# ShingoNishimoto/gnss_sim_receiver

Measured on AMD Instinct MI355X. Metric: IF Msamples/sec processed & tracked-channels sustained @1/2/4/8 GPU, higher is better.
Workload: dtype f32

## Files before the change

gnss_sim_receiver_amd/csrc/trk_fast.hip:

```cpp
#include <algorithm>
#include <cstdlib>
#include <type_traits>

#include "code_bits.h"
#include "corr_device.h"
#include "trk_engine.h"

#ifdef GNSSHIP_CORR_PROFILE
namespace gnsship {
namespace {
constexpr int kFProfEpochs = 16;
constexpr int kFProfFirst = 8;
constexpr int kFProfSlots = 88;
__device__ unsigned long long* g_trkf_prof = nullptr;
__shared__ int g_fprof_epoch;
__shared__ unsigned long long g_fprof_lds[kFProfEpochs * kFProfSlots];
#ifndef GNSSHIP_PROF_MASK
#define GNSSHIP_PROF_MASK 0xffffffffffffffffull
#endif
__device__ __forceinline__ constexpr bool prof_on(int k) { return ((GNSSHIP_PROF_MASK) >> (k < 63 ? k : 63)) & 1ull; }
__device__ __forceinline__ void trkf_prof_stamp(int e, int k)
{
    if (!prof_on(k)) return;
    const int r = e - kFProfFirst;
// ... 48 lines not shown
#pragma clang fp contract(off)

namespace gnsship {
namespace {

#ifndef GNSSHIP_FAST_WAVES
#define GNSSHIP_FAST_WAVES 8
#endif
#ifndef GNSSHIP_THRU_WAVES
#define GNSSHIP_THRU_WAVES 6
#endif
#ifndef GNSSHIP_FAST_WAVES_LONG
#define GNSSHIP_FAST_WAVES_LONG 8
#endif
constexpr int kFWaves = GNSSHIP_FAST_WAVES;
constexpr int kFWavesLong = GNSSHIP_FAST_WAVES_LONG;
constexpr int kLongEpoch = 10000;
#ifndef GNSSHIP_PRE_DISC
#define GNSSHIP_PRE_DISC 1
#endif
#ifndef GNSSHIP_ROLE_PLAN_LONG
#define GNSSHIP_ROLE_PLAN_LONG 3
#endif
#ifndef GNSSHIP_ROLE_PLAN
#define GNSSHIP_ROLE_PLAN 0
#endif
template <int NTT>
constexpr int acc_waves() { return (2 * NTT + 3) / 4; }
template <int NTT, int W>
constexpr int n_producers() { return W - 2 - acc_waves<NTT>(); }
constexpr int kMaxAccWaves = 4;
static_assert(kFWaves - 4 >= 1 && GNSSHIP_THRU_WAVES - 4 >= 1, "trk_fast needs at least one producer wave");
constexpr int kRoleControl = 0, kRoleReplay = 1, kRoleProducer = 2, kRoleAccum = 3;
#define GNSSHIP_PROBE(NAME)                                                  \
    do {                                                                     \
        _Pragma("unroll") for (int pr_ = 0; pr_ < (NAME); pr_++) __builtin_amdgcn_s_sleep(4); \
    } while (0)
#ifndef GNSSHIP_DELAY_ACC
#define GNSSHIP_DELAY_ACC 0
#endif
#ifndef GNSSHIP_DELAY_PROD
#define GNSSHIP_DELAY_PROD 0
#endif
#ifndef GNSSHIP_DELAY_REPLAY
#define GNSSHIP_DELAY_REPLAY 0
#endif
#ifndef GNSSHIP_DELAY_LOOP
#define GNSSHIP_DELAY_LOOP 0
#endif
#ifndef GNSSHIP_POLL_SLEEP
#define GNSSHIP_POLL_SLEEP 0
#endif
constexpr uint64_t kSlotEmpty = ~0ull;

struct FJob {
    int64_t off;
    float rem_code, code_step;
    float shifts[5];
    float dz_re, dz_im;
    float rem_carr, step;
    int32_t runnable, in_margin, M, S, tail, steady;
    int32_t narrow;
};

typedef uint32_t u4v __attribute__((ext_vector_type(4)));
constexpr uint32_t kJobRunnable = 1u, kJobInMargin = 2u, kJobSteady = 4u, kJobNarrow = 8u;
struct alignas(16) FJobLds {
    uint32_t w[8];
};
__device__ __forceinline__ void job_store_a(FJobLds& s, int64_t off, uint32_t flags, float rem_code, float code_step)
{
    const uint64_t o = static_cast<uint64_t>(off);
    *reinterpret_cast<u4v*>(&s.w[0]) = u4v{static_cast<uint32_t>(o), (static_cast<uint32_t>(o >> 32) & 0x00ffffffu) | (flags << 24),
        __builtin_bit_cast(uint32_t, rem_code), __builtin_bit_cast(uint32_t, code_step)};
}
__device__ __forceinline__ void job_store_b(FJobLds& s, float rem_carr, float step, float dz_re, float dz_im)
{
    *reinterpret_cast<u4v*>(&s.w[4]) = u4v{__builtin_bit_cast(uint32_t, rem_carr), __builtin_bit_cast(uint32_t, step),
        __builtin_bit_cast(uint32_t, dz_re), __builtin_bit_cast(uint32_t, dz_im)};
}
__device__ __forceinline__ void job_store_carr(FJobLds& s, float rem_carr, float step) { *reinterpret_cast<f2*>(&s.w[4]) = f2{rem_carr, step}; }
__device__ __forceinline__ void job_store_dz(FJobLds& s, f2 dz) { *reinterpret_cast<f2*>(&s.w[6]) = dz; }

struct SpecArgs {
    double step_d, rate;
    int64_t if_num;
    float rem_prev;
    int32_t n_pred;
};

struct alignas(16) SpecPred {
    float rem, step, dz_re, dz_im;
};

struct FShared {
    FJobLds job;
    float taps[2][2 * kMaxTaps + 2];
    int32_t taps_seq[kMaxAccWaves];
    gnsship_trk_dump_record drec;
    double coh;
    int32_t seed_seq;
    int32_t job_seq;
    int32_t pre_seq;
    int32_t lock_seq;
    int32_t locked;
    int32_t tail_seq;
// ... 98 lines not shown
            GNSSHIP_PSTEP_ASM(GNSSHIP_PSTEP("%[x]", "%[w]") GNSSHIP_PSTEP("%[w]", "%[x]"));
    } else if constexpr (N == 3) {
        if constexpr (STORE)
            GNSSHIP_PSTEP_ASM(GNSSHIP_PSTEP("%[x]", "%[w]") GNSSHIP_ST GNSSHIP_PSTEP("%[w]", "%[v]") GNSSHIP_PSTEP("%[v]", "%[x]"));
        else
            GNSSHIP_PSTEP_ASM(GNSSHIP_PSTEP("%[x]", "%[w]") GNSSHIP_PSTEP("%[w]", "%[v]") GNSSHIP_PSTEP("%[v]", "%[x]"));
    } else {
        if constexpr (STORE)
            GNSSHIP_PSTEP_ASM(GNSSHIP_PSTEP("%[x]", "%[w]") GNSSHIP_ST GNSSHIP_PSTEP("%[w]", "%[v]") GNSSHIP_PSTEP("%[v]", "%[w]")
                    GNSSHIP_PSTEP("%[w]", "%[x]"));
        else
            GNSSHIP_PSTEP_ASM(GNSSHIP_PSTEP("%[x]", "%[w]") GNSSHIP_PSTEP("%[w]", "%[v]") GNSSHIP_PSTEP("%[v]", "%[w]") GNSSHIP_PSTEP("%[w]", "%[x]"));
    }
    return x;
}
#undef GNSSHIP_ST
#undef GNSSHIP_PSTEP_ASM

#define GNSSHIP_PS(A, B) GNSSHIP_PSTEP("%[" #A "]", "%[" #B "]")
#define GNSSHIP_TST(A, OFF) "ds_write_b32 %[p], %[" #A "] offset:" #OFF "\n\t"
#define GNSSHIP_TASK8(A, B, OFF)                                                                                            \
    GNSSHIP_PS(A, B) GNSSHIP_TST(A, OFF) GNSSHIP_PS(B, A) GNSSHIP_PS(A, B) GNSSHIP_PS(B, A) GNSSHIP_PS(A, B) GNSSHIP_PS(B, A) \
        GNSSHIP_PS(A, B) GNSSHIP_PS(B, A)
__device__ __forceinline__ float pblock64_g8(float x, float c, float k2, uint32_t lds_off)
{
    float t, u, w;
    asm volatile(GNSSHIP_PS(x, w) GNSSHIP_PS(w, x) GNSSHIP_PS(x, w) GNSSHIP_PS(w, x) GNSSHIP_PS(x, w) GNSSHIP_PS(w, x)
                     GNSSHIP_PS(x, w) GNSSHIP_TASK8(w, x, 128) GNSSHIP_TASK8(w, x, 256) GNSSHIP_TASK8(w, x, 384) GNSSHIP_TASK8(w, x, 512)
                         GNSSHIP_TASK8(w, x, 640) GNSSHIP_TASK8(w, x, 768) GNSSHIP_TASK8(w, x, 896) "v_mov_b32 %[x], %[w]\n\t"
                 : [x] "+v"(x), [t] "=&v"(t), [u] "=&v"(u), [w] "=&v"(w)
                 : [c] "s"(c), [k2] "v"(k2), [p] "v"(lds_off)
                 : "memory");
    return x;
}
#undef GNSSHIP_TST
#undef GNSSHIP_TASK8
#undef GNSSHIP_PS
template <int N>
__device__ __forceinline__ float ppow(float x, float c, float k2)
{
    if constexpr (N >= 4) return ppow<N - 4>(pstep<4, false>(x, c, k2, 0), c, k2);
    else if constexpr (N > 0) return pstep<N, false>(x, c, k2, 0);
    else return x;
}
#undef GNSSHIP_PSTEP

__device__ __forceinline__ float pnormalise(float x)
{
    const float s = __fmul_rn(x, x);
    const float o = __builtin_bit_cast(float, __builtin_amdgcn_mov_dpp(__builtin_bit_cast(int, s), 0xB1, 0xF, 0xF, false));
    return __fdiv_rn(x, sqrt_rn_f32(__fadd_rn(s, o)));
}

template <int G, bool SRING>
__device__ __forceinline__ float fast_replay(float x, float c, float k2, int M, int S, int tail, uint64_t* __restrict__ Zs, int rs, int lane)
{
    static_assert(G % 4 == 0 && G >= 4 && G <= 64, "task length");
    constexpr int kTB = 64 / G;
    if (S <= 0) return x;
    c = __builtin_bit_cast(float, __builtin_amdgcn_readfirstlane(__builtin_bit_cast(int, c)));
    const uint32_t base = static_cast<uint32_t>(reinterpret_cast<uintptr_t>(Zs)) + 4u * static_cast<uint32_t>(lane);
    uint32_t off = base;
    constexpr uint32_t kSlotRow = kAvxLanes * sizeof(uint64_t);
    uint32_t* const half0 = reinterpret_cast<uint32_t*>(Zs) + lane;
    int ts = 0;
    if constexpr (!SRING) {
        const int full = (S - 1) / kTB;
#pragma unroll 1
        for (int b = 0; b < full; b++) {
            if constexpr (G == 8 && kSlotRow == 128) {
                x = pblock64_g8(pnormalise(pstep<1, true>(x, c, k2, off)), c, k2, off);
                off += kTB * kSlotRow;
            } else {
#pragma unroll
                for (int q = 0; q < kTB; q++) {
                    if (q == 0)
                        x = ppow<G - 1>(pnormalise(pstep<1, true>(x, c, k2, off)), c, k2);
                    else
                        x = ppow<G - 4>(pstep<4, true>(x, c, k2, off), c, k2);
                    off += kSlotRow;
                }
            }
        }
        if (full * kTB < S - 1) {
            x = ppow<G - 1>(pnormalise(pstep<1, true>(x, c, k2, off)), c, k2);
            off += kSlotRow;
#pragma unroll 1
            for (int t = full * kTB + 1; t < S - 1; t++) {
                x = ppow<G - 4>(pstep<4, true>(x, c, k2, off), c, k2);
                off += kSlotRow;
            }
        }
        ts = S - 1;
    } else {
        int t = 0;
        if constexpr (G == 8 && kSlotRow == 128) {
            if (rs % kTB == 0) {
                const int full = (S - 1) / kTB;
#pragma unroll 1
                for (int b = 0; b < full; b++, t += kTB) {
                    const int ts0 = t % rs;
                    if (t >= rs) {
                        bool busy = true;
                        while (busy) {
                            uint32_t v[kTB];
#pragma unroll
                            for (int q = 0; q < kTB; q++) v[q] = __hip_atomic_load(half0 + 2 * kAvxLanes * (ts0 + q), __ATOMIC_RELAXED, __HIP_MEMORY_SCOPE_WORKGROUP);
                            busy = false;
#pragma unroll
                            for (int q = 0; q < kTB; q++) busy = busy || v[q] != ~0u;
                            if (busy) __builtin_amdgcn_s_sleep(GNSSHIP_POLL_SLEEP);
                        }
                    }
                    off = base + static_cast<uint32_t>(ts0) * kSlotRow;
                    x = pblock64_g8(pnormalise(pstep<1, true>(x, c, k2, off)), c, k2, off);
                }
            }
        }
        ts = t % rs;
        off = base + static_cast<uint32_t>(ts) * kSlotRow;
#pragma unroll 1
        for (; t < S - 1; t++) {
            if (t >= rs)
                while (__hip_atomic_load(half0 + 2 * kAvxLanes * ts, __ATOMIC_RELAXED, __HIP_MEMORY_SCOPE_WORKGROUP) != ~0u) __builtin_amdgcn_s_sleep(GNSSHIP_POLL_SLEEP);
            if (t % kTB == 0)
                x = ppow<G - 1>(pnormalise(pstep<1, true>(x, c, k2, off)), c, k2);
            else
                x = ppow<G - 4>(pstep<4, true>(x, c, k2, off), c, k2);
            ts = ts + 1 == rs ? 0 : ts + 1;
            off = base + static_cast<uint32_t>(ts) * kSlotRow;
        }
        if (S - 1 >= rs)
            while (__hip_atomic_load(half0 + 2 * kAvxLanes * ts, __ATOMIC_RELAXED, __HIP_MEMORY_SCOPE_WORKGROUP) != ~0u) __builtin_amdgcn_s_sleep(GNSSHIP_POLL_SLEEP);
    }
    __hip_atomic_store(half0 + 2 * kAvxLanes * ts, __builtin_bit_cast(uint32_t, x), __ATOMIC_RELAXED, __HIP_MEMORY_SCOPE_WORKGROUP);
    if (tail > 0) {
        for (int m = G * (S - 1); m < M; m++) {
            x = pstep<1, false>(x, c, k2, 0);
// ... 10 lines not shown
{
    if constexpr (PACKED) return code_chip<IN_MARGIN>(code, L, sn, sh, rem);
    else return code_at<IN_MARGIN>(code, L, sn, sh, rem);
}
__host__ __device__ constexpr int fast_code_stride(bool packed, int code_cap_floats)
{
    return packed ? (lane_code_words(code_cap_floats) + 3) / 4 * 4 : code_cap_floats;
}

template <int NT, bool DATA, bool IN_MARGIN, int G, bool FULL, bool PACKED>
__device__ __forceinline__ void group_codes(CodePtr<PACKED> __restrict__ code0, CodePtr<PACKED> __restrict__ code1, int L, int n0, int cnt, float step,
    float rem, const float (&shifts)[NT], float (&cv)[G][NT + (DATA ? 1 : 0)])
{
    float fn = static_cast<float>(n0);
    const float fn0 = fn;
#pragma unroll
    for (int i = 0; i < G; i++) {
        const bool on = FULL || i < cnt;
        const float sn = __fmul_rn(step, on ? fn : fn0);
#pragma unroll
        for (int q = 0; q < NT; q++) cv[i][q] = chip_at<PACKED, IN_MARGIN>(code0, L, sn, shifts[q], rem);
        if constexpr (DATA) cv[i][NT] = chip_at<PACKED, IN_MARGIN>(code1, L, sn, 0.0f, rem);
        fn += static_cast<float>(kAvxLanes);
    }
}

typedef float f4 __attribute__((ext_vector_type(4)));

template <int NTT, int G>
struct ProdLayout {
    static constexpr int kJ = 4 * G;
    static constexpr int kRow = kJ + 4;
    static constexpr int kSlot = kAvxLanes * kRow;
    static constexpr int kGroup = 2 * NTT * kSlot;
};

template <int NTT, int G, bool FULL, class PL>
__device__ __forceinline__ void store_products4(float* __restrict__ pdst, int i0, int cnt, const f2 (&a)[4], const float (&cv)[G][NTT])
{
    f4 q[2 * NTT];
#pragma unroll
    for (int u = 0; u < 4; u++) {
        const bool on = FULL || i0 + u < cnt;
#pragma unroll
        for (int t = 0; t < NTT; t++) {
            q[2 * t][u] = on ? __fmul_rn(a[u].x, cv[i0 + u][t]) : -0.0f;
            q[2 * t + 1][u] = on ? __fmul_rn(a[u].y, cv[i0 + u][t]) : -0.0f;
        }
    }
#pragma unroll
    for (int sl = 0; sl < 2 * NTT; sl++) *reinterpret_cast<f4*>(pdst + sl * PL::kSlot + i0) = q[sl];
}

template <int FMT, int NTT, int G, bool FULL, class PL>
__device__ __forceinline__ void group_phasors(i4v span, f2 z, f2 dz, bool renorm, int n0, int cnt, float* __restrict__ pdst, const float (&cv)[G][NTT],
    f2 (&xa)[G < 8 ? G : 8], f2 (&xb)[G < 8 ? G : 8])
{
    constexpr int SB = sample_bytes<FMT>();
    constexpr int kB = G < 8 ? G : 8;
    static_assert(kB % 4 == 0, "16-byte product stores");
#pragma unroll 1
    for (int i0 = 0; i0 < G; i0 += kB) {
        if (i0 + kB < G) {
#pragma unroll
            for (int u = 0; u < kB; u++) xb[u] = load_sample<FMT>(span, (n0 + kAvxLanes * (i0 + kB + u)) * SB, 0);
        }
#pragma unroll
        for (int h = 0; h < kB; h += 4) {
            f2 a[4];
#pragma unroll
            for (int u = 0; u < 4; u++) {
                const int i = i0 + h + u;
                a[u] = cmul_exact_pk(xa[h + u], z);
                f2 zn = cmul_exact_s(z, dz);
                if (i == 0 && renorm) zn = normalise_avx(zn);
                z = zn;
            }
            store_products4<NTT, G, FULL, PL>(pdst, i0 + h, cnt, a, cv);
        }
        if (i0 + kB < G) {
#pragma unroll
            for (int u = 0; u < kB; u++) xa[u] = xb[u];
        }
    }
}

template <int FMT, int NT, bool DATA, bool IN_MARGIN, int G, int W, bool PACKED>
__device__ __forceinline__ void fast_produce(const FJob& job, i4v span, CodePtr<PACKED> __restrict__ code0, CodePtr<PACKED> __restrict__ code1, int L,
    uint64_t* __restrict__ Zs, int rs, float* __restrict__ Pp, int rg, int32_t* ready, const int32_t* acc_groups, int gbase, int lane, int pw, int pe,
    f2 (&xa)[G < 8 ? G : 8], float (&cv)[G][NT + (DATA ? 1 : 0)])
{
    constexpr int SB = sample_bytes<FMT>();
    constexpr int NTT = NT + (DATA ? 1 : 0);
    constexpr int NP = n_producers<NTT, W>();
    constexpr int NA = acc_waves<NTT>();
    using PL = ProdLayout<NTT, G>;
    constexpr int kB = G < 8 ? G : 8;
    const int M = job.M, S = job.S;
    const int n_groups = (S + 3) / 4;
    const f2 dz = f2{job.dz_re, job.dz_im};
    const float step = job.code_step, rem = job.rem_code;
    float shifts[NT];
#pragma unroll
    for (int q = 0; q < NT; q++) shifts[q] = job.shifts[q];
    const int tl = lane >> 4, l = lane & (kAvxLanes - 1);
    f2 xb[kB];
    int rslot = pw % rg;
    const int rstep = NP % rg;
    unsigned long long w_ring = 0, w_slot = 0, w_codes = 0, w_prod = 0;
    [[maybe_unused]] const unsigned long long t_run = GNSSHIP_FCLOCK();
    for (int g = pw; g < n_groups; g += NP) {
        const int t = 4 * g + tl;
        const bool active = t < S;
        const int m_lo = G * (active ? t : 0);
        const int cnt = active ? min(G, M - m_lo) : 0;
        const int n0 = kAvxLanes * m_lo + l;
        const bool full = 4 * g + 4 <= S && G * (4 * g + 4) <= M;
        const unsigned long long tA = GNSSHIP_FCLOCK();
#pragma unroll
        for (int u = 0; u < kB; u++) xa[u] = load_sample<FMT>(span, (n0 + kAvxLanes * u) * SB, 0);
        if (full)
            group_codes<NT, DATA, IN_MARGIN, G, true, PACKED>(code0, code1, L, n0, G, step, rem, shifts, cv);
        else
            group_codes<NT, DATA, IN_MARGIN, G, false, PACKED>(code0, code1, L, n0, cnt, step, rem, shifts, cv);
#ifdef GNSSHIP_CORR_PROFILE
        for (int i = 0; i < G; i++)
            for (int q = 0; q < NTT; q++) asm volatile("" ::"v"(cv[i][q]));
#endif
        w_codes += GNSSHIP_FCLOCK() - tA;
        const unsigned long long t0 = GNSSHIP_FCLOCK();
        if (g >= rg) {
#pragma unroll
            for (int a = 0; a < NA; a++) lds_wait_ge(acc_groups + a, gbase + g - rg + 1);
        }
        const unsigned long long t1 = GNSSHIP_FCLOCK();
        w_ring += t1 - t0;
        uint64_t* slot = Zs + (active ? t % rs : 0) * kAvxLanes + l;
        uint64_t v = kSlotEmpty;
        if (active) {
            while (static_cast<uint32_t>(v = load_slot(slot)) == ~0u || static_cast<uint32_t>(v >> 32) == ~0u) __builtin_amdgcn_s_sleep(GNSSHIP_POLL_SLEEP);
            store_slot(slot, __builtin_bit_cast(f2, kSlotEmpty));
        }
        w_slot += GNSSHIP_FCLOCK() - t1;
        if (g == pw && pw == 0) GNSSHIP_FSTAMP(pe, 30);
        if (g + NP >= n_groups && pw == 1) GNSSHIP_FSTAMP(pe, 31);
        const f2 z = active ? __builtin_bit_cast(f2, v) : f2{0.0f, 0.0f};
        const bool renorm = ((G * t) & 63) == 0;
        float* pdst = Pp + static_cast<size_t>(rslot) * PL::kGroup + l * PL::kRow + G * tl;
        const unsigned long long tB = GNSSHIP_FCLOCK();
        if (full)
            group_phasors<FMT, NTT, G, true, PL>(span, z, dz, renorm, n0, G, pdst, cv, xa, xb);
        else
            group_phasors<FMT, NTT, G, false, PL>(span, z, dz, renorm, n0, cnt, pdst, cv, xa, xb);
        GNSSHIP_PROBE(GNSSHIP_DELAY_PROD);
        if (lane == 0) lds_release_store(ready + 2 * rslot, gbase + g + 1);
        w_prod += GNSSHIP_FCLOCK() - tB;
        if (g < 8) GNSSHIP_FSTAMP(pe, 48 + g);
        rslot += rstep;
        if (rslot >= rg) rslot -= rg;
    }
    if (pw == 0) {
        GNSSHIP_FVAL(pe, 41, w_ring);
        GNSSHIP_FVAL(pe, 42, w_slot);
        GNSSHIP_FVAL(pe, 43, GNSSHIP_FCLOCK() - t_run);
        GNSSHIP_FVAL(pe, 79, w_codes);
        GNSSHIP_FVAL(pe, 80, w_prod);
    }
}

template <int NTT>
constexpr int acc_slots() { return (2 * NTT + 4 * acc_waves<NTT>() - 1) / (4 * acc_waves<NTT>()); }
template <int NTT>
__device__ __forceinline__ int acc_slot(int a, int r, int k) { return 4 * (a + acc_waves<NTT>() * k) + r; }

template <int NTT, int G>
__device__ __forceinline__ void fast_accumulate(const float* __restrict__ Pp, int rg, const int32_t* ready, int32_t* acc_done, int gbase, int S,
    int lane, int a, float (&acc)[acc_slots<NTT>()], int pe)
{
    using PL = ProdLayout<NTT, G>;
    constexpr int NS = acc_slots<NTT>();
    constexpr int kQ = PL::kJ / 4;
    const int l = lane & (kAvxLanes - 1), r = lane >> 4;
    const int n_groups = (S + 3) / 4;
    int off[NS];
#pragma unroll
    for (int k = 0; k < NS; k++) {
        acc[k] = 0.0f;
        off[k] = min(acc_slot<NTT>(a, r, k), 2 * NTT - 1) * PL::kSlot + l * PL::kRow;
    }
    unsigned long long w_flag = 0;
    [[maybe_unused]] const unsigned long long t_run = GNSSHIP_FCLOCK();
    int rslot = 0;
    for (int g = 0; g < n_groups; g++) {
        const unsigned long long t0 = GNSSHIP_FCLOCK();
        lds_wait_eq(ready + 2 * rslot, gbase + g + 1);
        const float* src = Pp + static_cast<size_t>(rslot) * PL::kGroup;
        f4 v[kQ][NS];
#pragma unroll
        for (int q = 0; q < kQ; q++)
#pragma unroll
            for (int k = 0; k < NS; k++) v[q][k] = *reinterpret_cast<const f4*>(src + off[k] + 4 * q);
        w_flag += GNSSHIP_FCLOCK() - t0;
#pragma unroll
        for (int q = 0; q < kQ; q++)
#pragma unroll
            for (int k = 0; k < NS; k++)
#pragma unroll
                for (int u = 0; u < 4; u++) acc[k] = __fadd_rn(acc[k], v[q][k][u]);
        if (g == 0) GNSSHIP_FSTAMP(pe, 28);
        if (g == n_groups - 1) GNSSHIP_FSTAMP(pe, 29);
#pragma unroll
        for (int k = 0; k < NS; k++) asm volatile("" ::"v"(acc[k]) : "memory");
        GNSSHIP_PROBE(GNSSHIP_DELAY_ACC);
        if (lane == 0) __hip_atomic_store(acc_done, gbase + g + 1, __ATOMIC_RELAXED, __HIP_MEMORY_SCOPE_WORKGROUP);
        rslot = rslot + 1 == rg ? 0 : rslot + 1;
    }
    if (a < 2) {
        GNSSHIP_FVAL(pe, 44 + 2 * a, w_flag);
        GNSSHIP_FVAL(pe, 45 + 2 * a, GNSSHIP_FCLOCK() - t_run);
    }
}

__device__ __forceinline__ float avx_chain_sum(float d)
{
    float s = d + dpp_mov<0x12C>(d);
    s = s + dpp_mov<0x128>(d);
    s = s + dpp_mov<0x124>(d);
    float r = 0.0f + s;
    r = r + dpp_mov<0x101>(s);
    r = r + dpp_mov<0x102>(s);
    r = r + dpp_mov<0x103>(s);
    return r;
}

template <int FMT, int NT, bool DATA, bool IN_MARGIN, bool PACKED>
__device__ __forceinline__ void fast_tail_products(const FJob& job, i4v span, CodePtr<PACKED> __restrict__ code0, CodePtr<PACKED> __restrict__ code1, int L,
    const f2* T, int lane, f2 (*tp)[kMaxTaps + 1])
{
    constexpr int SB = sample_bytes<FMT>();
    if (lane >= job.tail) return;
    const int n = kAvxLanes * job.M + lane;
    const f2 x = load_sample<FMT>(span, n * SB, 0);
    const f2 wo = cmul_exact(x, T[lane]);
    const float sn = __fmul_rn(job.code_step, static_cast<float>(n));
#pragma unroll
    for (int q = 0; q < NT; q++) {
        const float c = chip_at<PACKED, IN_MARGIN>(code0, L, sn, job.shifts[q], job.rem_code);
        tp[lane][q] = wo * f2{c, c};
    }
    if constexpr (DATA) {
        const float c = chip_at<PACKED, IN_MARGIN>(code1, L, sn, 0.0f, job.rem_code);
        tp[lane][NT] = wo * f2{c, c};
    }
}

__device__ __forceinline__ void stage_code_f(float* dst, const CodeDesc& cd, int nthreads)
{
    const int nq = padded_code_quads(cd.len);
    const float4* src = reinterpret_cast<const float4*>(cd.ptr - kCodeMargin);
    float4* d4 = reinterpret_cast<float4*>(dst);
    for (int q = threadIdx.x; q < nq; q += nthreads) d4[q] = src[q];
}

// ... 23 lines not shown
__device__ __forceinline__ void derive_all(float step, float rem, int lane, f2& inc, f2& dz, f2& zinit)
{
    float ss, cs, sr, cr;
    glibc_sincosf(-step, &ss, &cs);
    glibc_sincosf(rem, &sr, &cr);
    inc = f2{cs, ss};
    const f2 p0 = f2{cr, -sr};
    f2 w = p0, z = p0, d = inc;
#pragma unroll
    for (int i = 0; i < kAvxLanes - 1; i++) {
        w = cmul_exact_sc(w, inc);
        if (i < 4) d = cmul_exact_sc(d, d);
        z = i + 1 == (lane >> 1) ? w : z;
    }
    dz = normalise_avx(d);
    zinit = z;
}

__device__ __forceinline__ uint64_t uni64(uint64_t v)
{
    const uint32_t lo = __builtin_amdgcn_readfirstlane(static_cast<uint32_t>(v)), hi = __builtin_amdgcn_readfirstlane(static_cast<uint32_t>(v >> 32));
    return (static_cast<uint64_t>(hi) << 32) | lo;
}

__device__ __forceinline__ f2 derive_chains(float rem, f2 inc, int lane)
{
    float sfn, cfn;
    glibc_sincosf(rem, &sfn, &cfn);
    const f2 p0 = f2{cfn, -sfn};
    f2 w = p0, z = p0;
#pragma unroll
    for (int i = 0; i < kAvxLanes - 1; i++) {
        w = cmul_exact_sc(w, inc);
        z = i + 1 == (lane >> 1) ? w : z;
    }
    return z;
}

template <int FMT, int NT, bool DATA, int G, bool THRU, bool SRING, int W, bool PACKED>
__global__ __launch_bounds__(W * kWave, (fast_waves_per_simd<THRU, W>())) void trk_fast_kernel(const TrkParams* __restrict__ pk, TrkChannel* __restrict__ chans,
    const CodeDesc* __restrict__ codes, int n_codes, const void* __restrict__ samples, uint64_t buf_first, int64_t buf_len, int max_rounds,
    int n_chans, int code_cap_floats, int rs, int rg, gnsship_trk_epoch* __restrict__ rec, gnsship_trk_dump_record* __restrict__ dump,
    gnsship_trk_corr_trace* __restrict__ trace, int* __restrict__ ran_count)
{
    constexpr int NTT = NT + (DATA ? 1 : 0);
    constexpr int kFWaves = W;
    constexpr int kFThreads = kFWaves * kWave;
    static_assert(acc_waves<NTT>() <= kMaxAccWaves && n_producers<NTT, kFWaves>() >= 1, "trk_fast wave roles");
    extern __shared__ __attribute__((aligned(16))) float lds[];
    __shared__ TrkChannel sc;
    __shared__ FShared sh;
    __shared__ int32_t skip;
    __shared__ f2 tailz[kAvxLanes];
    const int ch = blockIdx.x;
    const int tid = threadIdx.x, lane = tid & (kWave - 1), wave = __builtin_amdgcn_readfirstlane(tid >> 6);
    const TrkParams& k = *pk;
    {
        const int* src = reinterpret_cast<const int*>(chans + ch);
        int* dst = reinterpret_cast<int*>(&sc);
        for (int i = tid; i < static_cast<int>(sizeof(TrkChannel) / 4); i += kFThreads) dst[i] = src[i];
    }
    uint64_t* Zs = reinterpret_cast<uint64_t*>(lds);
    float* code0 = reinterpret_cast<float*>(Zs + static_cast<size_t>(rs) * kAvxLanes);
    const int code_stride = fast_code_stride(PACKED, code_cap_floats);
    float* code1 = code0 + code_stride;
    float* Pp = code0 + (DATA ? 2 : 1) * code_stride;
    int32_t* ready = reinterpret_cast<int32_t*>(Pp + static_cast<size_t>(rg) * ProdLayout<NTT, G>::kGroup);
    for (int i = tid; i < rs * kAvxLanes; i += kFThreads) Zs[i] = kSlotEmpty;
    for (int i = tid; i < 2 * rg; i += kFThreads) ready[i] = 0;
    __shared__ int32_t simd_of[kFWaves];
    if (lane == 0) simd_of[wave] = static_cast<int32_t>((__builtin_amdgcn_s_getreg(4 | (31 << 11)) >> 4) & 3);
#ifdef GNSSHIP_CORR_PROFILE
    for (int i = tid; i < kFProfEpochs * kFProfSlots; i += kFThreads) g_fprof_lds[i] = 0;
#endif
    __syncthreads();
    constexpr int NA = acc_waves<NTT>();
    int role = kRoleProducer, pw = 0;
    {
        auto count = [&](int sd) {
            int c = 0;
            for (int w = 0; w < kFWaves; w++) c += (simd_of[w] & 3) == sd ? 1 : 0;
            return c;
        };
        auto assign = [&](int plan) __attribute__((always_inline)) {
            int nacc = 0, nprod = 0, nsimd = 0;
            bool ctl = false, rep = false;
            for (int cc = 1; cc <= kFWaves; cc++)
                for (int sd = 0; sd < 4; sd++) {
                    if (count(sd) != cc) continue;
                    bool first = true;
                    for (int w = 0; w < kFWaves; w++) {
                        if ((simd_of[w] & 3) != sd) continue;
                        int rl, idx = 0;
                        if (plan == 3) {
                            if (nsimd == 0 && !rep) {
                                rl = kRoleReplay;
                                rep = true;
                            } else if (nsimd == 1 && nacc < NA) {
                                rl = kRoleAccum;
                                idx = nacc++;
                            } else if (nsimd == 2 && !ctl) {
                                rl = kRoleControl;
                                ctl = true;
                            } else if (nsimd >= 2 && nacc < NA) {
                                rl = kRoleAccum;
                                idx = nacc++;
                            } else if (nsimd >= 3 && !ctl) {
                                rl = kRoleControl;
                                ctl = true;
                            } else {
                                rl = kRoleProducer;
                                idx = nprod++;
                            }
                        } else if (plan == 2) {
                            if (nsimd == 0 && !rep) {
                                rl = kRoleReplay;
                                rep = true;
                            } else if (nsimd == 0 && !ctl) {
                                rl = kRoleControl;
                                ctl = true;
                            } else if (nsimd >= 1 && nacc < NA) {
// ... 194 lines not shown
        }
    };
    if (role == kRoleControl) make_seed(0);
    int e_done = 0;
    bool cancel = false;
    if (role == kRoleReplay) {
        float shc[5];
        int sh_nw = -1;
        for (int e = 0;; e++) {
            FJob job;
                bool spec = false;
                SpecArgs sp{};
                while (__hip_atomic_load(&sh.seed_seq, __ATOMIC_RELAXED, __HIP_MEMORY_SCOPE_WORKGROUP) < e + 1) {
                    if (__hip_atomic_load(&sh.step_seq, __ATOMIC_RELAXED, __HIP_MEMORY_SCOPE_WORKGROUP) >= e + 1) {
                        sp.step_d = __builtin_bit_cast(double, uni64(__builtin_bit_cast(uint64_t, sh.spec.step_d)));
                        sp.rate = __builtin_bit_cast(double, uni64(__builtin_bit_cast(uint64_t, sh.spec.rate)));
                        sp.if_num = static_cast<int64_t>(uni64(static_cast<uint64_t>(sh.spec.if_num)));
                        sp.rem_prev = __builtin_bit_cast(float, __builtin_amdgcn_readfirstlane(__builtin_bit_cast(int, sh.spec.rem_prev)));
                        sp.n_pred = __builtin_amdgcn_readfirstlane(sh.spec.n_pred);
                        spec = true;
                        break;
                    }
                    __builtin_amdgcn_s_sleep(GNSSHIP_POLL_SLEEP);
                }
                __builtin_amdgcn_fence(__ATOMIC_ACQUIRE, "workgroup");
                GNSSHIP_FSTAMP(e, 0);
    #ifdef GNSSHIP_CORR_PROFILE
                if (lane == 0) g_fprof_epoch = e;
    #endif
                f2 zinit = f2{0.0f, 0.0f}, inc = f2{1.0f, 0.0f}, dz = f2{1.0f, 0.0f};
                float step_pre = 0.0f;
                bool published = false;
                float xl = 0.0f;
                if (spec) step_pre = static_cast<float>(sp.step_d + if_step);
                if (SRING && spec) derive_step(step_pre, inc, dz);
                if (!SRING && spec) {
                    float rem_pred = carr_rem_next(sp.rem_prev, carr_advance(sp.step_d, sp.rate, static_cast<double>(sp.n_pred)));
                    if (has_if) {
                        const int64_t ifn = (sp.if_num + kp.if_mod * static_cast<int64_t>(sp.n_pred)) % kp.fs_int;
                        const double ifc = static_cast<double>(ifn) / static_cast<double>(kp.fs_int);
                        rem_pred = static_cast<float>(fmod_2pi(static_cast<double>(rem_pred) + kTwoPi * ifc));
                    }
                    derive_all(step_pre, rem_pred, lane, inc, dz, zinit);
                    GNSSHIP_FSTAMP(e, 35);
                    GNSSHIP_PROBE(GNSSHIP_DELAY_REPLAY);
                    if (lane == 0) {
                        sh.pred.rem = rem_pred;
                        sh.pred.step = step_pre;
                        sh.pred.dz_re = dz.x;
                        sh.pred.dz_im = dz.y;
                        publish_seq(&sh.pred_seq, e + 1);
                    }
                    xl = (lane & 1) ? zinit.y : zinit.x;
                    if (lane < 2 * kAvxLanes) xl = fast_replay<G, false>(xl, dz.x, (lane & 1) ? dz.y : -dz.y, M, S, tail, Zs, rs, lane);
                    GNSSHIP_FSTAMP(e, 34);
                    wait_seq(&sh.seed_seq, e + 1);
                    const int v = __builtin_amdgcn_readfirstlane(sh.verdict);
                    int status = (v >> 2) == e + 1 ? (v & 3) : 3;
                    if (status == 3) {
                        const FJob sd = read_job(shc, sh_nw);
                        status = 2;
                        if (sd.runnable && __builtin_bit_cast(uint32_t, sd.step) == __builtin_bit_cast(uint32_t, step_pre) &&
                            __builtin_bit_cast(uint32_t, sd.rem_carr) == __builtin_bit_cast(uint32_t, rem_pred)) {
                            if (lane == 0) {
                                job_store_dz(sh.job, dz);
                                publish_seq(&sh.job_seq, e + 1);
                            }
                            status = 1;
                        }
                    }
                    GNSSHIP_FVAL(e, 78, static_cast<unsigned long long>(status));
                    if (status == 1) {
                        published = true;
                    } else {
                        for (int i = lane; i < S * kAvxLanes; i += kWave) Zs[i] = kSlotEmpty;
                    }
                    GNSSHIP_FSTAMP(e, 36);
                }
                if (!published) {
                    wait_seq(&sh.seed_seq, e + 1);
                    const FJob sd = read_job(shc, sh_nw);
                    if (sd.runnable) {
                        if (!(spec && __builtin_bit_cast(uint32_t, sd.step) == __builtin_bit_cast(uint32_t, step_pre))) derive_step(sd.step, inc, dz);
                        zinit = derive_chains(sd.rem_carr, inc, lane);
                        if (lane == 0) job_store_dz(sh.job, dz);
                    }
                    if (lane == 0) publish_seq(&sh.job_seq, e + 1);
                    if (!sd.runnable) break;
                }
                GNSSHIP_FSTAMP(e, 1);
                GNSSHIP_FCLK(e, 12);
                job = read_job(shc, sh_nw);
                if (!published) {
                    xl = (lane & 1) ? zinit.y : zinit.x;
                    if (lane < 2 * kAvxLanes) xl = fast_replay<G, SRING>(xl, job.dz_re, (lane & 1) ? job.dz_im : -job.dz_im, M, S, tail, Zs, rs, lane);
                }
                if (tail > 0) {
                    const i4v span = sample_span<FMT>(samples, job.off, N);
                    const f2 zl = f2{__builtin_bit_cast(float, __builtin_amdgcn_readlane(__builtin_bit_cast(int, xl), 0)),
                        __builtin_bit_cast(float, __builtin_amdgcn_readlane(__builtin_bit_cast(int, xl), 1))};
                    if (lane == 0) {
                        f2 p = normalise_avx(zl);
                        for (int j = 0; j < tail; j++) {
                            tailz[j] = p;
                            p = cmul_exact(p, inc);
                        }
                    }
                    if (job.in_margin)
                        fast_tail_products<FMT, NT, DATA, true, PACKED>(job, span, c0, c1, L, tailz, lane, sh.tailp);
                    else
                        fast_tail_products<FMT, NT, DATA, false, PACKED>(job, span, c0, c1, L, tailz, lane, sh.tailp);
                    if (lane == 0) publish_seq(&sh.tail_seq, e + 1);
                }
                GNSSHIP_FSTAMP(e, 2);
                GNSSHIP_FCLK(e, 13);
        }
    } else if (role == kRoleProducer) {
        f2 xa[G < 8 ? G : 8];
        float cv[G][NTT];
        bool lost = false;
        float shc[5];
        int sh_nw = -1;
        const double coh_steady = k.code_period * static_cast<double>(k.sync[uni(sc.geo)].extend);
        for (int e = 0;; e++) {
            const int gbase = e * n_groups;
            wait_seq(&sh.job_seq, e + 1);
            const FJob job = read_job(shc, sh_nw);
            if (!job.runnable) break;
            const i4v span = sample_span<FMT>(samples, job.off, N);
            if (job.in_margin)
                fast_produce<FMT, NT, DATA, true, G, kFWaves, PACKED>(job, span, c0, c1, L, Zs, rs, Pp, rg, ready, sh.acc_groups, gbase, lane, pw, e, xa, cv);
            else
                fast_produce<FMT, NT, DATA, false, G, kFWaves, PACKED>(job, span, c0, c1, L, Zs, rs, Pp, rg, ready, sh.acc_groups, gbase, lane, pw, e, xa, cv);
            if (pw < 2) GNSSHIP_FSTAMP(e, 3 + pw);
            if (pw == 0) {
                bool locked = true;
                if (kSteadyForm && job.steady) {
#pragma unroll
                    for (int a = 0; a < NA; a++) wait_seq(&sh.taps_seq[a], e + 1);
                    if (lane == 0) {
                        GNSSHIP_FSTAMP(e, 8);
                        if (!lost) {
                            const float* tp = sh.taps[e & 1] + (k.veml ? 2 : 0);
                            sc.p[0] = __fadd_rn(0.0f, __fmul_rn(1.0f, tp[2]));
                            sc.p[1] = __fadd_rn(0.0f, __fmul_rn(1.0f, tp[3]));
                            locked = lock_status(k, sc, coh_steady);
                        }
                        sh.locked = locked ? 1 : 0;
                        GNSSHIP_FSTAMP(e, 26);
                        publish_seq(&sh.lock_seq, e + 1);
                    }
                } else {
                    wait_seq(&sh.pre_seq, e + 1);
                    const double coh = sh.coh;
                    if (lane == 0) {
                        GNSSHIP_FSTAMP(e, 8);
                        locked = !(coh > 0.0 && !lock_status(k, sc, coh));
                        sh.locked = locked ? 1 : 0;
                        GNSSHIP_FSTAMP(e, 26);
                        publish_seq(&sh.lock_seq, e + 1);
                    }
                }
                lost = __builtin_amdgcn_readfirstlane(locked ? 0 : 1) != 0;
            }
        }
    } else if (role == kRoleAccum) {
        float shc[5];
        int sh_nw = -1;
        for (int e = 0;; e++) {
            const int gbase = e * n_groups;
            wait_seq(&sh.job_seq, e + 1);
            const FJob job = read_job(shc, sh_nw);
            if (!job.runnable) break;
            {
                constexpr int NS = acc_slots<NTT>();
                float acc[NS];
                GNSSHIP_FSTAMP(e, 27);
                fast_accumulate<NTT, G>(Pp, rg, ready, &sh.acc_groups[pw], gbase, S, lane, pw, acc, e);
                GNSSHIP_FSTAMP(e, 5);
                const int r = lane >> 4;
    #pragma unroll
                for (int kk = 0; kk < NS; kk++) acc[kk] = avx_chain_sum(acc[kk]);
                if (job.tail > 0) {
                    wait_seq(&sh.tail_seq, e + 1);
                    for (int j = 0; j < job.tail; j++) {
    #pragma unroll
// ... 283 lines not shown
    }
    __syncthreads();
#ifdef GNSSHIP_CORR_PROFILE
    if (g_trkf_prof)
        for (int i = tid; i < kFProfEpochs * kFProfSlots; i += kFThreads) g_trkf_prof[static_cast<size_t>(blockIdx.x) * kFProfEpochs * kFProfSlots + i] = g_fprof_lds[i];
#endif
    {
        const int* src = reinterpret_cast<const int*>(&sc);
        int* dst = reinterpret_cast<int*>(chans + ch);
        for (int i = tid; i < static_cast<int>(sizeof(TrkChannel) / 4); i += kFThreads) dst[i] = src[i];
    }
}

}

#ifdef GNSSHIP_CORR_PROFILE
}
extern "C" int gnsship_debug_trk_fast_profile(void* dev_buf)
{
    return hipMemcpyToSymbol(HIP_SYMBOL(gnsship::g_trkf_prof), &dev_buf, sizeof(void*)) == hipSuccess ? 0 : -3;
}
namespace gnsship {
#endif

static int device_cus()
{
    static int cache[64] = {0};
    int dev = 0;
    if (hipGetDevice(&dev) != hipSuccess || dev < 0 || dev >= 64) return 256;
    if (cache[dev] == 0) {
        int n = 0;
        cache[dev] = (hipDeviceGetAttribute(&n, hipDeviceAttributeMultiprocessorCount, dev) == hipSuccess && n > 0) ? n : 256;
    }
    return cache[dev];
}

static bool fast_thru(int n_chans)
{
    if (const char* env = std::getenv("GNSSHIP_TRK_THRU")) return env[0] == '1';
    return n_chans > device_cus();
}

struct FastPlan {
    size_t bytes = 0;
    int G = 8, rs = 0, rg = 0;
    bool packed = false;
};
#ifndef GNSSHIP_FAST_G
#define GNSSHIP_FAST_G 8
#endif
constexpr int kFastG = GNSSHIP_FAST_G;
constexpr int kFastSlotRingGroups = 16;
constexpr int kFastMinRingGroups = 4;
constexpr size_t kFastMaxSlotBytes = 48 * 1024;
static bool fast_packed_only_layout(const TrkParams& p) { return p.n_taps == 3 && p.jobs_per_channel > 1; }
static bool fast_packed_layout(const TrkParams& p, bool codes_binary)
{
    if (fast_packed_only_layout(p)) return true;
    if (!p.single_code_bits || !codes_binary || p.n_taps != 3 || p.jobs_per_channel > 1) return false;
    const char* env = std::getenv("GNSSHIP_TRK_FAST_PACKED");
    return !(env && env[0] == '0');
}

static FastPlan fast_plan(const TrkParams& p, int code_cap_floats, int n_chans, bool codes_binary)
{
    FastPlan f;
    f.packed = fast_packed_layout(p, codes_binary);
    if (p.n_taps == 5 && fast_thru(n_chans)) return f;
    const int N = static_cast<int>(p.conf.vector_length);
    const int M = N / kAvxLanes;
    const int G = kFastG;
    const int S = std::max(1, (M + G - 1) / G);
    const int n_groups = (S + 3) / 4;
    const int ntt = p.n_taps + (p.jobs_per_channel > 1 ? 1 : 0);
    const size_t codes = static_cast<size_t>(p.jobs_per_channel > 1 ? 2 : 1) * fast_code_stride(f.packed, code_cap_floats) * sizeof(float);
    const size_t slot_b = kAvxLanes * sizeof(uint64_t);
    const size_t group_b = static_cast<size_t>(2 * ntt) * kAvxLanes * (4 * G + 4) * sizeof(float) + 2 * sizeof(int32_t);
    size_t budget = fast_thru(n_chans) ? 72 * 1024 : kTrkPersistMaxLds;
    if (const char* env = std::getenv("GNSSHIP_TRK_FAST_LDS"))
        budget = std::min(budget, static_cast<size_t>(std::atol(env)) * 1024);
    auto fit = [&](int rs) -> int {
        const size_t used = codes + static_cast<size_t>(rs) * slot_b;
        if (used >= budget) return 0;
        const int rg = static_cast<int>(std::min<size_t>((budget - used) / group_b, static_cast<size_t>(n_groups)));
        return rg >= std::min(2, n_groups) ? rg : 0;
    };
    int rs = S, rg = static_cast<size_t>(S) * slot_b <= kFastMaxSlotBytes ? fit(S) : 0;
    if (rg < std::min(n_groups, kFastMinRingGroups) && S > 4 * kFastSlotRingGroups) {
        const int rg2 = std::min(fit(4 * kFastSlotRingGroups), kFastSlotRingGroups);
        if (rg2 > rg) {
            rs = 4 * kFastSlotRingGroups;
            rg = rg2;
        }
    }
    if (rg == 0) return f;
    f.G = G;
    f.rs = rs;
    f.rg = rg;
    f.bytes = codes + static_cast<size_t>(rs) * slot_b + static_cast<size_t>(rg) * group_b;
    return f;
}

bool trk_fast_thru(int n_chans) { return fast_thru(n_chans); }
int trk_device_cus() { return device_cus(); }

bool trk_fast_supported(const TrkParams& p, int code_cap_floats, int n_chans, bool codes_binary)
{
// ... 82 lines not shown
```

Before: 695.5.

## Publish replay-normalised phasors to LDS so producers skip renormalisation

The replay wave now writes its normalised phasor at each 64-iteration block boundary into a new LDS row array (Zn). Producers poll that row at renorm points and take the exact value instead of calling normalise_avx themselves, which takes a sqrt/divide off the producer critical path. In exchange there is extra LDS space, a spin-wait dependency on the replay wave, and extra slot resets. A profiling stamp for the first accumulator groups is also added.

```diff
diff --git a/gnss_sim_receiver_amd/csrc/trk_fast.hip b/gnss_sim_receiver_amd/csrc/trk_fast.hip
--- a/gnss_sim_receiver_amd/csrc/trk_fast.hip
+++ b/gnss_sim_receiver_amd/csrc/trk_fast.hip
@@ -124,6 +124,8 @@
 #define GNSSHIP_POLL_SLEEP 0
 #endif
 constexpr uint64_t kSlotEmpty = ~0ull;
+constexpr size_t kFastMaxSlotBytes = 48 * 1024;
+constexpr int kZnRows = static_cast<int>(kFastMaxSlotBytes / (kAvxLanes * sizeof(uint64_t)) / 8);
 
 struct FJob {
     int64_t off;
@@ -328,9 +330,12 @@
     return __fdiv_rn(x, sqrt_rn_f32(__fadd_rn(s, o)));
 }
 
-template <int G, bool SRING>
-__device__ __forceinline__ float fast_replay(float x, float c, float k2, int M, int S, int tail, uint64_t* __restrict__ Zs, int rs, int lane)
-{
+template <int G, bool SRING, bool ZN>
+__device__ __forceinline__ float fast_replay(float x, float c, float k2, int M, int S, int tail, uint64_t* __restrict__ Zs, int rs, int lane,
+    uint64_t* __restrict__ Zn)
+{
+    static_assert(!ZN || (!SRING && G == 8), "Zn: one row per 64-iteration block of 8 tasks");
+    [[maybe_unused]] uint32_t* zn_half = reinterpret_cast<uint32_t*>(Zn) + lane;
     static_assert(G % 4 == 0 && G >= 4 && G <= 64, "task length");
     constexpr int kTB = 64 / G;
     if (S <= 0) return x;
@@ -345,7 +350,12 @@
 #pragma unroll 1
         for (int b = 0; b < full; b++) {
             if constexpr (G == 8 && kSlotRow == 128) {
-                x = pblock64_g8(pnormalise(pstep<1, true>(x, c, k2, off)), c, k2, off);
+                x = pnormalise(pstep<1, true>(x, c, k2, off));
+                if constexpr (ZN) {
+                    __hip_atomic_store(zn_half, __builtin_bit_cast(uint32_t, x), __ATOMIC_RELAXED, __HIP_MEMORY_SCOPE_WORKGROUP);
+                    zn_half += 2 * kAvxLanes;
+                }
+                x = pblock64_g8(x, c, k2, off);
                 off += kTB * kSlotRow;
             } else {
 #pragma unroll
@@ -359,7 +369,9 @@
             }
         }
         if (full * kTB < S - 1) {
-            x = ppow<G - 1>(pnormalise(pstep<1, true>(x, c, k2, off)), c, k2);
+            x = pnormalise(pstep<1, true>(x, c, k2, off));
+            if constexpr (ZN) __hip_atomic_store(zn_half, __builtin_bit_cast(uint32_t, x), __ATOMIC_RELAXED, __HIP_MEMORY_SCOPE_WORKGROUP);
+            x = ppow<G - 1>(x, c, k2);
             off += kSlotRow;
 #pragma unroll 1
             for (int t = full * kTB + 1; t < S - 1; t++) {
@@ -476,8 +488,8 @@
     for (int sl = 0; sl < 2 * NTT; sl++) *reinterpret_cast<f4*>(pdst + sl * PL::kSlot + i0) = q[sl];
 }
 
-template <int FMT, int NTT, int G, bool FULL, class PL>
-__device__ __forceinline__ void group_phasors(i4v span, f2 z, f2 dz, bool renorm, int n0, int cnt, float* __restrict__ pdst, const float (&cv)[G][NTT],
+template <int FMT, int NTT, int G, bool FULL, bool ZN, class PL>
+__device__ __forceinline__ void group_phasors(i4v span, f2 z, f2 dz, bool renorm, f2 zq, bool take_zn, int n0, int cnt, float* __restrict__ pdst, const float (&cv)[G][NTT],
     f2 (&xa)[G < 8 ? G : 8], f2 (&xb)[G < 8 ? G : 8])
 {
     constexpr int SB = sample_bytes<FMT>();
@@ -497,7 +509,13 @@
                 const int i = i0 + h + u;
                 a[u] = cmul_exact_pk(xa[h + u], z);
                 f2 zn = cmul_exact_s(z, dz);
-                if (i == 0 && renorm) zn = normalise_avx(zn);
+                if constexpr (ZN && FULL) {
+                    if (i == 0 && renorm) zn = zq;
+                } else if constexpr (ZN) {
+                    if (i == 0 && renorm) zn = take_zn ? zq : normalise_avx(zn);
+                } else {
+                    if (i == 0 && renorm) zn = normalise_avx(zn);
+                }
                 z = zn;
             }
             store_products4<NTT, G, FULL, PL>(pdst, i0 + h, cnt, a, cv);
@@ -509,9 +527,9 @@
     }
 }
 
-template <int FMT, int NT, bool DATA, bool IN_MARGIN, int G, int W, bool PACKED>
+template <int FMT, int NT, bool DATA, bool IN_MARGIN, int G, int W, bool PACKED, bool ZN>
 __device__ __forceinline__ void fast_produce(const FJob& job, i4v span, CodePtr<PACKED> __restrict__ code0, CodePtr<PACKED> __restrict__ code1, int L,
-    uint64_t* __restrict__ Zs, int rs, float* __restrict__ Pp, int rg, int32_t* ready, const int32_t* acc_groups, int gbase, int lane, int pw, int pe,
+    uint64_t* __restrict__ Zs, uint64_t* __restrict__ Zn, int rs, float* __restrict__ Pp, int rg, int32_t* ready, const int32_t* acc_groups, int gbase, int lane, int pw, int pe,
     f2 (&xa)[G < 8 ? G : 8], float (&cv)[G][NT + (DATA ? 1 : 0)])
 {
     constexpr int SB = sample_bytes<FMT>();
@@ -570,12 +588,24 @@
         if (g + NP >= n_groups && pw == 1) GNSSHIP_FSTAMP(pe, 31);
         const f2 z = active ? __builtin_bit_cast(f2, v) : f2{0.0f, 0.0f};
         const bool renorm = ((G * t) & 63) == 0;
+        f2 zq = f2{0.0f, 0.0f};
+        bool take_zn = false;
+        if constexpr (ZN) {
+            take_zn = active && renorm && t < S - 1;
+            if (take_zn) {
+                uint64_t* nslot = Zn + (t >> 3) * kAvxLanes + l;
+                uint64_t w = kSlotEmpty;
+                while (static_cast<uint32_t>(w = load_slot(nslot)) == ~0u || static_cast<uint32_t>(w >> 32) == ~0u) __builtin_amdgcn_s_sleep(GNSSHIP_POLL_SLEEP);
+                store_slot(nslot, __builtin_bit_cast(f2, kSlotEmpty));
+                zq = __builtin_bit_cast(f2, w);
+            }
+        }
         float* pdst = Pp + static_cast<size_t>(rslot) * PL::kGroup + l * PL::kRow + G * tl;
         const unsigned long long tB = GNSSHIP_FCLOCK();
         if (full)
-            group_phasors<FMT, NTT, G, true, PL>(span, z, dz, renorm, n0, G, pdst, cv, xa, xb);
+            group_phasors<FMT, NTT, G, true, ZN, PL>(span, z, dz, renorm, zq, take_zn, n0, G, pdst, cv, xa, xb);
         else
-            group_phasors<FMT, NTT, G, false, PL>(span, z, dz, renorm, n0, cnt, pdst, cv, xa, xb);
+            group_phasors<FMT, NTT, G, false, ZN, PL>(span, z, dz, renorm, zq, take_zn, n0, cnt, pdst, cv, xa, xb);
         GNSSHIP_PROBE(GNSSHIP_DELAY_PROD);
         if (lane == 0) lds_release_store(ready + 2 * rslot, gbase + g + 1);
         w_prod += GNSSHIP_FCLOCK() - tB;
@@ -633,6 +663,7 @@
                 for (int u = 0; u < 4; u++) acc[k] = __fadd_rn(acc[k], v[q][k][u]);
         if (g == 0) GNSSHIP_FSTAMP(pe, 28);
         if (g == n_groups - 1) GNSSHIP_FSTAMP(pe, 29);
+        if (g < 8) GNSSHIP_FSTAMP(pe, 64 + g);
 #pragma unroll
         for (int k = 0; k < NS; k++) asm volatile("" ::"v"(acc[k]) : "memory");
         GNSSHIP_PROBE(GNSSHIP_DELAY_ACC);
@@ -762,6 +793,9 @@
     __shared__ FShared sh;
     __shared__ int32_t skip;
     __shared__ f2 tailz[kAvxLanes];
+    constexpr bool kZn = !SRING && !THRU && G == 8;
+    __shared__ uint64_t zn_rows[kZn ? kZnRows * kAvxLanes : 1];
+    uint64_t* const Zn = zn_rows;
     const int ch = blockIdx.x;
     const int tid = threadIdx.x, lane = tid & (kWave - 1), wave = __builtin_amdgcn_readfirstlane(tid >> 6);
     const TrkParams& k = *pk;
@@ -777,6 +811,8 @@
     float* Pp = code0 + (DATA ? 2 : 1) * code_stride;
     int32_t* ready = reinterpret_cast<int32_t*>(Pp + static_cast<size_t>(rg) * ProdLayout<NTT, G>::kGroup);
     for (int i = tid; i < rs * kAvxLanes; i += kFThreads) Zs[i] = kSlotEmpty;
+    if constexpr (kZn)
+        for (int i = tid; i < kZnRows * kAvxLanes; i += kFThreads) Zn[i] = kSlotEmpty;
     for (int i = tid; i < 2 * rg; i += kFThreads) ready[i] = 0;
     __shared__ int32_t simd_of[kFWaves];
     if (lane == 0) simd_of[wave] = static_cast<int32_t>((__builtin_amdgcn_s_getreg(4 | (31 << 11)) >> 4) & 3);
@@ -1077,7 +1113,7 @@
                         publish_seq(&sh.pred_seq, e + 1);
                     }
                     xl = (lane & 1) ? zinit.y : zinit.x;
-                    if (lane < 2 * kAvxLanes) xl = fast_replay<G, false>(xl, dz.x, (lane & 1) ? dz.y : -dz.y, M, S, tail, Zs, rs, lane);
+                    if (lane < 2 * kAvxLanes) xl = fast_replay<G, false, kZn>(xl, dz.x, (lane & 1) ? dz.y : -dz.y, M, S, tail, Zs, rs, lane, Zn);
                     GNSSHIP_FSTAMP(e, 34);
                     wait_seq(&sh.seed_seq, e + 1);
                     const int v = __builtin_amdgcn_readfirstlane(sh.verdict);
@@ -1099,6 +1135,8 @@
                         published = true;
                     } else {
                         for (int i = lane; i < S * kAvxLanes; i += kWave) Zs[i] = kSlotEmpty;
+                        if constexpr (kZn)
+                            for (int i = lane; i < (S + 7) / 8 * kAvxLanes; i += kWave) Zn[i] = kSlotEmpty;
                     }
                     GNSSHIP_FSTAMP(e, 36);
                 }
@@ -1118,7 +1156,7 @@
                 job = read_job(shc, sh_nw);
                 if (!published) {
                     xl = (lane & 1) ? zinit.y : zinit.x;
-                    if (lane < 2 * kAvxLanes) xl = fast_replay<G, SRING>(xl, job.dz_re, (lane & 1) ? job.dz_im : -job.dz_im, M, S, tail, Zs, rs, lane);
+                    if (lane < 2 * kAvxLanes) xl = fast_replay<G, SRING, kZn>(xl, job.dz_re, (lane & 1) ? job.dz_im : -job.dz_im, M, S, tail, Zs, rs, lane, Zn);
                 }
                 if (tail > 0) {
                     const i4v span = sample_span<FMT>(samples, job.off, N);
@@ -1154,9 +1192,9 @@
             if (!job.runnable) break;
             const i4v span = sample_span<FMT>(samples, job.off, N);
             if (job.in_margin)
-                fast_produce<FMT, NT, DATA, true, G, kFWaves, PACKED>(job, span, c0, c1, L, Zs, rs, Pp, rg, ready, sh.acc_groups, gbase, lane, pw, e, xa, cv);
+                fast_produce<FMT, NT, DATA, true, G, kFWaves, PACKED, kZn>(job, span, c0, c1, L, Zs, Zn, rs, Pp, rg, ready, sh.acc_groups, gbase, lane, pw, e, xa, cv);
             else
-                fast_produce<FMT, NT, DATA, false, G, kFWaves, PACKED>(job, span, c0, c1, L, Zs, rs, Pp, rg, ready, sh.acc_groups, gbase, lane, pw, e, xa, cv);
+                fast_produce<FMT, NT, DATA, false, G, kFWaves, PACKED, kZn>(job, span, c0, c1, L, Zs, Zn, rs, Pp, rg, ready, sh.acc_groups, gbase, lane, pw, e, xa, cv);
             if (pw < 2) GNSSHIP_FSTAMP(e, 3 + pw);
             if (pw == 0) {
                 bool locked = true;
@@ -1546,7 +1584,6 @@
 constexpr int kFastG = GNSSHIP_FAST_G;
 constexpr int kFastSlotRingGroups = 16;
 constexpr int kFastMinRingGroups = 4;
-constexpr size_t kFastMaxSlotBytes = 48 * 1024;
 static bool fast_packed_only_layout(const TrkParams& p) { return p.n_taps == 3 && p.jobs_per_channel > 1; }
 static bool fast_packed_layout(const TrkParams& p, bool codes_binary)
 {
```

Result: no change. 701.5 (median of 6 runs) (+0.9%).
